# yisol/IDM-VTON

Measured on AMD Instinct MI355X. Metric: try-on images/sec at 768x1024, 30 DDIM steps, guidance 2.0, higher is better.
Workload: dtype bf16; 1 GPU; BASELINE.json configs[1]: 768x1024, 30 steps, batch 2/GPU, guidance 2.0, bf16 storage / fp32 accumulate, scheduler ddim, hipGraph on, GarmentNet batched over 6 timesteps, GarmentNet(block b+1)||TryonNet(block b) two-stream overlap on; images_per_call=2, parallelism=dp1 (image shards, one start-up RCCL weight broadcast), rccl_ranks=1

## Files before the change

### idm-vton_amd/csrc/norm.hip

```cpp
#include <cstdlib>
#include "common.cuh"

template <typename T, int NCH, bool X32, int RPW>
__global__ __launch_bounds__(256) void layernorm_kernel(const idmvton_layernorm_args a) {
    typedef typename VT<T>::v8 v8;
    const int lane = threadIdx.x & 63;
    const int row0 = (blockIdx.x * 4 + (threadIdx.x >> 6)) * RPW;
    if (row0 >= a.rows) return;
    const int nchunk = a.C >> 3;
    const T* gamma = (const T*)a.gamma;
    const T* beta = (const T*)a.beta;
    v8 gm[NCH], bt_[NCH];
#pragma unroll
    for (int i = 0; i < NCH; ++i) {
        const int c = lane + 64 * i;
        if (c < nchunk) { gm[i] = *(const v8*)(gamma + c * 8); bt_[i] = *(const v8*)(beta + c * 8); }
    }
    float v[RPW][NCH][8];
    float s[RPW];
#pragma unroll
    for (int r = 0; r < RPW; ++r) {
        const int row = row0 + r < a.rows ? row0 + r : a.rows - 1;
        const T* x = (const T*)a.x + (size_t)row * a.ldx;
        const float* xf = (const float*)a.x + (size_t)row * a.ldx;
// ... 92 lines not shown
template <typename T, bool X32> struct GnLoad {
    typedef typename VT<T>::v8 v8;
    struct raw { v8 t; };
    static __device__ __forceinline__ raw ld(const void* base, size_t idx) { raw r; r.t = *(const v8*)((const T*)base + idx); return r; }
    static __device__ __forceinline__ float get(const raw& r, int j) { return (float)r.t[j]; }
};
template <typename T> struct GnLoad<T, true> {
    struct raw { float4 a, b; };
    static __device__ __forceinline__ raw ld(const void* base, size_t idx) {
        raw r; const float4* p = (const float4*)((const float*)base + idx); r.a = p[0]; r.b = p[1]; return r;
    }
    static __device__ __forceinline__ float get(const raw& r, int j) {
        return j == 0 ? r.a.x : j == 1 ? r.a.y : j == 2 ? r.a.z : j == 3 ? r.a.w : j == 4 ? r.b.x : j == 5 ? r.b.y : j == 6 ? r.b.z : r.b.w;
    }
};

template <typename T, bool X32>
__global__ __launch_bounds__(256) void gn_stats_kernel(const idmvton_groupnorm_args a, int pix_per_block, int nblk) {
    typedef GnLoad<T, X32> L;
    __shared__ float red_s[GN_MAXC], red_q[GN_MAXC];
    const int b = blockIdx.y;
    const int nchunk = a.C >> 3;
    const int tpp = 256 / nchunk > 0 ? 256 / nchunk : 1;
    const int chunk = threadIdx.x % nchunk, psub = threadIdx.x / nchunk;
    const int p0 = blockIdx.x * pix_per_block;
    const int p1 = min(p0 + pix_per_block, a.HW);
    for (int cb = chunk; cb < nchunk; cb += 256) {
        const int c0 = cb * 8;
        const void* src; int pitch, coff;
        if (c0 < a.C1) { src = a.x; pitch = a.C1; coff = c0; }
        else { src = a.x2; pitch = a.C - a.C1; coff = c0 - a.C1; }
        float s[8], q[8];
#pragma unroll
        for (int j = 0; j < 8; ++j) { s[j] = 0.f; q[j] = 0.f; }
        if (psub < tpp) {
            int pix = p0 + psub;
            for (; pix + 3 * tpp < p1; pix += 4 * tpp) {
                typename L::raw t[4];
#pragma unroll
                for (int u4 = 0; u4 < 4; ++u4) t[u4] = L::ld(src, ((size_t)b * a.HW + pix + u4 * tpp) * pitch + coff);
#pragma unroll
                for (int u4 = 0; u4 < 4; ++u4)
#pragma unroll
                    for (int j = 0; j < 8; ++j) { const float f = L::get(t[u4], j); s[j] += f; q[j] += f * f; }
            }
            for (; pix < p1; pix += tpp) {
                const typename L::raw t = L::ld(src, ((size_t)b * a.HW + pix) * pitch + coff);
#pragma unroll
                for (int j = 0; j < 8; ++j) { const float f = L::get(t, j); s[j] += f; q[j] += f * f; }
            }
#pragma unroll
            for (int j = 0; j < 8; ++j) { red_s[psub * a.C + c0 + j] = s[j]; red_q[psub * a.C + c0 + j] = q[j]; }
        }
    }
    __syncthreads();
    for (int c = threadIdx.x; c < a.C; c += 256) {
        float ss = red_s[c], qq = red_q[c];
        for (int p = 1; p < tpp; ++p) { ss += red_s[p * a.C + c]; qq += red_q[p * a.C + c]; }
        red_s[c] = ss; red_q[c] = qq;
    }
    __syncthreads();
    const int cpg = a.C / a.groups;
    double* part = a.stats + (size_t)2 * a.B * a.groups;
    for (int g = threadIdx.x; g < a.groups; g += 256) {
        double ds = 0.0, dq = 0.0;
        for (int c = g * cpg; c < (g + 1) * cpg; ++c) { ds += (double)red_s[c]; dq += (double)red_q[c]; }
        double* dst = part + (((size_t)b * a.groups + g) * nblk + blockIdx.x) * 2;
        dst[0] = ds; dst[1] = dq;
    }
}

__global__ __launch_bounds__(64) void gn_finalize_kernel(double* stats, int bg, int nblk, double cnt, double eps) {
    const int i = blockIdx.x, lane = threadIdx.x;
    const double* part = stats + (size_t)2 * bg + (size_t)i * nblk * 2;
    double ds = 0.0, dq = 0.0;
    int k = lane;
    for (; k + 3 * 64 < nblk; k += 4 * 64) {
        double ps[4], pq[4];
#pragma unroll
        for (int u4 = 0; u4 < 4; ++u4) { ps[u4] = part[2 * (k + 64 * u4)]; pq[u4] = part[2 * (k + 64 * u4) + 1]; }
#pragma unroll
        for (int u4 = 0; u4 < 4; ++u4) { ds += ps[u4]; dq += pq[u4]; }
    }
    for (; k < nblk; k += 64) { ds += part[2 * k]; dq += part[2 * k + 1]; }
#pragma unroll
    for (int o = 32; o > 0; o >>= 1) { ds += __shfl_xor(ds, o); dq += __shfl_xor(dq, o); }
    if (lane == 0) {
        const double mean = ds / cnt;
        double var = dq / cnt - mean * mean;
        var = var > 0.0 ? var : 0.0;
        float* o = (float*)(stats + 2 * i);
        o[0] = (float)mean;
        o[1] = (float)(1.0 / sqrt(var + eps));
    }
}

template <typename T, bool PREC>
__global__ __launch_bounds__(256) void gn_apply_kernel(const idmvton_groupnorm_args a, int pix_per_block) {
    typedef typename VT<T>::v8 v8;
    typedef GnLoad<T, PREC> L;
    const int b = blockIdx.y;
    const int nchunk = a.C >> 3;
    const int tpp = 256 / nchunk > 0 ? 256 / nchunk : 1;
    const int chunk = threadIdx.x % nchunk, psub = threadIdx.x / nchunk;
    const int p0 = blockIdx.x * pix_per_block;
    const int p1 = min(p0 + pix_per_block, a.HW);
    const int cpg = a.C / a.groups;
    const int opitch = PREC ? 2 * a.C : a.C;
    for (int cb = chunk; cb < nchunk; cb += 256) {
        const int c0 = cb * 8;
        const void* src; int pitch, coff;
        if (c0 < a.C1) { src = a.x; pitch = a.C1; coff = c0; }
        else { src = a.x2; pitch = a.C - a.C1; coff = c0 - a.C1; }
        float sc[8], sh[8];
#pragma unroll
        for (int j = 0; j < 8; ++j) {
            const int c = c0 + j, g = c / cpg;
            const float2 mr = *(const float2*)(a.stats + ((size_t)b * a.groups + g) * 2);
            const float gm = PREC ? ((const float*)a.gamma)[c] : (float)((const T*)a.gamma)[c];
            const float bt = PREC ? ((const float*)a.beta)[c] : (float)((const T*)a.beta)[c];
            sc[j] = mr.y * gm;
            sh[j] = bt - mr.x * sc[j];
        }
        auto emit = [&](const typename L::raw& t, size_t row) {
            T* dst = (T*)a.y + row * opitch + c0;
            v8 o, lo;
#pragma unroll
            for (int j = 0; j < 8; ++j) {
                float f = L::get(t, j) * sc[j] + sh[j];
                if (a.silu) f = silu_f(f);
                o[j] = (T)f;
                if constexpr (PREC) lo[j] = (T)(f - (float)o[j]);
            }
            *(v8*)dst = o;
            if constexpr (PREC) *(v8*)(dst + a.C) = lo;
        };
        if (psub < tpp) {
            int pix = p0 + psub;
            for (; pix + 3 * tpp < p1; pix += 4 * tpp) {
                typename L::raw t[4];
#pragma unroll
                for (int u4 = 0; u4 < 4; ++u4) t[u4] = L::ld(src, ((size_t)b * a.HW + pix + u4 * tpp) * pitch + coff);
#pragma unroll
                for (int u4 = 0; u4 < 4; ++u4) emit(t[u4], (size_t)b * a.HW + pix + u4 * tpp);
            }
            for (; pix < p1; pix += tpp) {
                const size_t row = (size_t)b * a.HW + pix;
                emit(L::ld(src, row * pitch + coff), row);
            }
        }
    }
}

static void gn_geometry(const idmvton_groupnorm_args& a, int& nblk, int& ppb) {
    nblk = (2048 + a.B - 1) / a.B;
    ppb = (a.HW + nblk - 1) / nblk;
    const int nchunk = a.C >> 3;
    const int tpp = 256 / nchunk > 0 ? 256 / nchunk : 1;
    if (ppb < tpp * 4) ppb = tpp * 4;
    nblk = (a.HW + ppb - 1) / ppb;
}

template <typename T>
static int launch_gn(const idmvton_groupnorm_args& a, hipStream_t st) {
    int nblk, ppb;
    gn_geometry(a, nblk, ppb);
    const dim3 grid(nblk, a.B), block(256);
    const bool prec = a.flags != 0;
    if (prec) hipLaunchKernelGGL((gn_stats_kernel<T, true>), grid, block, 0, st, a, ppb, nblk);
    else hipLaunchKernelGGL((gn_stats_kernel<T, false>), grid, block, 0, st, a, ppb, nblk);
    hipLaunchKernelGGL(gn_finalize_kernel, dim3(a.B * a.groups), dim3(64), 0, st, a.stats, a.B * a.groups, nblk,
                       (double)(a.C / a.groups) * (double)a.HW, (double)a.eps);
    if (prec) hipLaunchKernelGGL((gn_apply_kernel<T, true>), grid, block, 0, st, a, ppb);
    else hipLaunchKernelGGL((gn_apply_kernel<T, false>), grid, block, 0, st, a, ppb);
    CHECK_LAUNCH("groupnorm");
    return IDMVTON_OK;
}

extern "C" int idmvton_groupnorm_stats_doubles(int B, int HW, int C, int groups) {
    if (B <= 0 || HW <= 0 || C < 8 || groups <= 0) return -1;
    idmvton_groupnorm_args a;
    a.B = B; a.HW = HW; a.C = C; a.groups = groups;
    int nblk, ppb;
    gn_geometry(a, nblk, ppb);
    return 2 * B * groups * (1 + nblk);
}

extern "C" int idmvton_groupnorm(const idmvton_groupnorm_args* a, void* stream) {
    CHECK_ARG(a != nullptr, IDMVTON_E_ARG, "groupnorm: null args");
    CHECK_ARG(a->dtype == IDMVTON_F16 || a->dtype == IDMVTON_BF16, IDMVTON_E_DTYPE, "groupnorm: dtype %d", a->dtype);
    CHECK_ARG(a->B > 0 && a->HW > 0 && a->C > 0 && a->groups > 0 && a->C % a->groups == 0 && a->C % 8 == 0 && a->C <= GN_MAXC,
              IDMVTON_E_SHAPE, "groupnorm: B=%d HW=%d C=%d groups=%d", a->B, a->HW, a->C, a->groups);
    CHECK_ARG(a->x && a->y && a->gamma && a->beta && a->stats, IDMVTON_E_ARG, "groupnorm: null pointer");
    CHECK_ARG(a->stats_doubles >= idmvton_groupnorm_stats_doubles(a->B, a->HW, a->C, a->groups), IDMVTON_E_SHAPE,
              "groupnorm: stats scratch holds %d doubles, needs %d", a->stats_doubles,
              idmvton_groupnorm_stats_doubles(a->B, a->HW, a->C, a->groups));
    CHECK_ARG(a->C1 > 0 && a->C1 <= a->C && a->C1 % 8 == 0 && (a->C1 == a->C || a->x2), IDMVTON_E_SHAPE, "groupnorm: C1=%d", a->C1);
    constexpr int PREC_FLAGS = IDMVTON_GN_X_F32 | IDMVTON_GN_Y_SPLIT | IDMVTON_GN_AFFINE_F32;
    CHECK_ARG(a->flags == 0 || a->flags == PREC_FLAGS, IDMVTON_E_ARG, "groupnorm: flags=%d (0, or the split-precision form X_F32 | Y_SPLIT | AFFINE_F32 = %d)", a->flags, PREC_FLAGS);
    if (a->flags) CHECK_ARG((((uintptr_t)a->gamma | (uintptr_t)a->beta) & 3) == 0, IDMVTON_E_ALIGN, "groupnorm: fp32 gamma / beta alignment");
    CHECK_ARG((((uintptr_t)a->x | (uintptr_t)a->x2 | (uintptr_t)a->y) & 15) == 0, IDMVTON_E_ALIGN, "groupnorm: pointer alignment");
    return a->dtype == IDMVTON_BF16 ? launch_gn<bf16_t>(*a, (hipStream_t)stream) : launch_gn<f16_t>(*a, (hipStream_t)stream);
}

template <typename T>
__global__ __launch_bounds__(256) void softmax_rows_kernel(T* x, int n, int ld, float scale, int nv) {
    typedef typename VT<T>::v8 v8;
    __shared__ float red[8];
    T* row = x + (size_t)blockIdx.x * ld;
    const int nchunk = n >> 3;
    const float sl = scale * 1.44269504088896341f;
    float mx = -3.0e38f;
    for (int c = threadIdx.x; c < nchunk; c += 256) {
        const v8 t = *(const v8*)(row + c * 8);
#pragma unroll
        for (int j = 0; j < 8; ++j) mx = fmaxf(mx, c * 8 + j < nv ? (float)t[j] : -3.0e38f);
    }
#pragma unroll
    for (int o = 32; o > 0; o >>= 1) mx = fmaxf(mx, __shfl_xor(mx, o));
    if ((threadIdx.x & 63) == 0) red[threadIdx.x >> 6] = mx;
    __syncthreads();
    mx = fmaxf(fmaxf(red[0], red[1]), fmaxf(red[2], red[3]));
    __syncthreads();
    float s = 0.f;
    for (int c = threadIdx.x; c < nchunk; c += 256) {
        const v8 t = *(const v8*)(row + c * 8);
#pragma unroll
        for (int j = 0; j < 8; ++j) s += c * 8 + j < nv ? __builtin_amdgcn_exp2f(((float)t[j] - mx) * sl) : 0.f;
    }
    s = wave_sum(s);
    if ((threadIdx.x & 63) == 0) red[4 + (threadIdx.x >> 6)] = s;
    __syncthreads();
    const float inv = 1.0f / (red[4] + red[5] + red[6] + red[7]);
    for (int c = threadIdx.x; c < nchunk; c += 256) {
        const v8 t = *(const v8*)(row + c * 8);
        v8 o;
#pragma unroll
        for (int j = 0; j < 8; ++j) o[j] = (T)(c * 8 + j < nv ? __builtin_amdgcn_exp2f(((float)t[j] - mx) * sl) * inv : 0.f);
        *(v8*)(row + c * 8) = o;
    }
}

template <typename T>
__global__ __launch_bounds__(256) void softmax_rows_split_kernel(const float* x, int n, int ld, float scale, T* y, int ldy, int nv) {
    typedef typename VT<T>::v8 v8;
    __shared__ float red[8];
    const float* row = x + (size_t)blockIdx.x * ld;
    T* yr = y + (size_t)blockIdx.x * ldy;
    const int nchunk = n >> 3;
    const float sl = scale * 1.44269504088896341f;
    float mx = -3.0e38f;
    for (int c = threadIdx.x; c < nchunk; c += 256) {
        const float4 t0 = *(const float4*)(row + c * 8), t1 = *(const float4*)(row + c * 8 + 4);
        const float v[8] = {t0.x, t0.y, t0.z, t0.w, t1.x, t1.y, t1.z, t1.w};
#pragma unroll
        for (int j = 0; j < 8; ++j) mx = fmaxf(mx, c * 8 + j < nv ? v[j] : -3.0e38f);
    }
#pragma unroll
    for (int o = 32; o > 0; o >>= 1) mx = fmaxf(mx, __shfl_xor(mx, o));
    if ((threadIdx.x & 63) == 0) red[threadIdx.x >> 6] = mx;
    __syncthreads();
    mx = fmaxf(fmaxf(red[0], red[1]), fmaxf(red[2], red[3]));
    __syncthreads();
    float s = 0.f;
    for (int c = threadIdx.x; c < nchunk; c += 256) {
        const float4 t0 = *(const float4*)(row + c * 8), t1 = *(const float4*)(row + c * 8 + 4);
        const float v[8] = {t0.x, t0.y, t0.z, t0.w, t1.x, t1.y, t1.z, t1.w};
#pragma unroll
        for (int j = 0; j < 8; ++j) s += c * 8 + j < nv ? __builtin_amdgcn_exp2f((v[j] - mx) * sl) : 0.f;
    }
    s = wave_sum(s);
    if ((threadIdx.x & 63) == 0) red[4 + (threadIdx.x >> 6)] = s;
    __syncthreads();
    const float inv = 1.0f / (red[4] + red[5] + red[6] + red[7]);
    for (int c = threadIdx.x; c < nchunk; c += 256) {
        const float4 t0 = *(const float4*)(row + c * 8), t1 = *(const float4*)(row + c * 8 + 4);
        const float v[8] = {t0.x, t0.y, t0.z, t0.w, t1.x, t1.y, t1.z, t1.w};
        v8 hi, lo;
#pragma unroll
        for (int j = 0; j < 8; ++j) {
            const float p = c * 8 + j < nv ? __builtin_amdgcn_exp2f((v[j] - mx) * sl) * inv : 0.f;
            hi[j] = (T)p;
            lo[j] = (T)(p - (float)hi[j]);
        }
        *(v8*)(yr + c * 8) = hi;
        *(v8*)(yr + n + c * 8) = lo;
    }
}

extern "C" int idmvton_softmax_rows(const idmvton_softmax_args* a, void* stream) {
    CHECK_ARG(a && a->x, IDMVTON_E_ARG, "softmax_rows: null pointer");
    CHECK_ARG(a->dtype == IDMVTON_F16 || a->dtype == IDMVTON_BF16, IDMVTON_E_DTYPE, "softmax_rows: dtype %d", a->dtype);
    CHECK_ARG(a->rows > 0 && a->n > 0 && a->n % 8 == 0 && (a->y_split || a->ld % 8 == 0) && a->ld >= a->n && ((uintptr_t)a->x & 15) == 0,
              IDMVTON_E_SHAPE, "softmax_rows: rows=%d n=%d ld=%d", a->rows, a->n, a->ld);
    const dim3 grid(a->rows), block(256);
    CHECK_ARG(a->n_valid >= 0 && a->n_valid <= a->n, IDMVTON_E_SHAPE, "softmax_rows: n_valid=%d n=%d", a->n_valid, a->n);
    const int nv = a->n_valid ? a->n_valid : a->n;
    if (a->y_split) {
        CHECK_ARG(a->ldy % 8 == 0 && a->ldy >= 2 * a->n && ((uintptr_t)a->y_split & 15) == 0 && a->ld % 4 == 0, IDMVTON_E_SHAPE, "softmax_rows: y_split ldy=%d n=%d", a->ldy, a->n);
        if (a->dtype == IDMVTON_BF16) hipLaunchKernelGGL((softmax_rows_split_kernel<bf16_t>), grid, block, 0, (hipStream_t)stream, (const float*)a->x, a->n, a->ld, a->scale, (bf16_t*)a->y_split, a->ldy, nv);
        else hipLaunchKernelGGL((softmax_rows_split_kernel<f16_t>), grid, block, 0, (hipStream_t)stream, (const float*)a->x, a->n, a->ld, a->scale, (f16_t*)a->y_split, a->ldy, nv);
        CHECK_LAUNCH("softmax_rows");
        return IDMVTON_OK;
    }
    if (a->dtype == IDMVTON_BF16) hipLaunchKernelGGL((softmax_rows_kernel<bf16_t>), grid, block, 0, (hipStream_t)stream, (bf16_t*)a->x, a->n, a->ld, a->scale, nv);
    else hipLaunchKernelGGL((softmax_rows_kernel<f16_t>), grid, block, 0, (hipStream_t)stream, (f16_t*)a->x, a->n, a->ld, a->scale, nv);
    CHECK_LAUNCH("softmax_rows");
    return IDMVTON_OK;
}
```

### idm-vton_amd/ffi.py

```python
import ctypes as C
import functools
import os

_HERE = os.path.dirname(os.path.abspath(__file__))
LIB_PATH = os.environ.get("IDMVTON_HIP_LIB") or os.path.join(_HERE, "libidmvton_hip.so")

F16, BF16, F32, F8E4M3 = 0, 1, 2, 3
EPI_NONE, EPI_GEGLU, EPI_GELU, EPI_QUICKGELU, EPI_XATTN = 0, 1, 2, 3, 4
ATTN_SELF, ATTN_CROSS = 0, 1
IO_RES_F32, IO_OUT_F32, IO_BIAS_F32, IO_OUT_F8 = 1, 2, 4, 8
GN_X_F32, GN_Y_SPLIT, GN_AFFINE_F32 = 1, 2, 4
LAYOUT_SPLIT, LAYOUT_NHWC_F32 = 1, 2
SPLIT_ACT, SPLIT_W3, SPLIT_W3T = 0, 1, 2
KVS_WIDEN_E4M3, KVS_COPY = 0, 1
MAX_SEG = 24
ABI_VERSION = 9

i32, u32, f32, vp = C.c_int32, C.c_uint32, C.c_float, C.c_void_p


class Seg(C.Structure):
    _fields_ = [("ptr", vp), ("bytes", u32), ("pitch", i32), ("coff", i32), ("len", i32), ("dy", i32), ("dx", i32)]


class XAttn(C.Structure):
    _fields_ = [("nseg", i32), ("k", vp * 2), ("ldk", i32 * 2), ("k_rows", i32 * 2), ("vt", vp * 2), ("ldvt", i32 * 2), ("nk", i32 * 2),
                ("tokens", i32), ("ip_scale", f32)]


class GemmConvArgs(C.Structure):
    _fields_ = [("dtype", i32), ("w", vp), ("N", i32), ("Ktot", i32), ("nseg", i32), ("seg", Seg * MAX_SEG),
                ("M", i32), ("Ho", i32), ("Wo", i32), ("Hi", i32), ("Wi", i32), ("stride", i32), ("ups", i32),
                ("out", vp), ("ldo", i32), ("bias", vp), ("rowbias", vp), ("rowbias_ld", i32),
                ("rows_per_group", i32), ("res", vp), ("ldr", i32), ("mode", i32), ("vt", vp), ("vt_n0", i32),
                ("vt_tokens", i32), ("tile_hint", i32), ("vt_perm", i32), ("io_flags", i32), ("xattn", C.POINTER(XAttn)),
                ("colscale_n", i32), ("colscale", f32), ("f8_out_scale", f32), ("f8_vt_scale", f32)]


class AttnArgs(C.Structure):
    _fields_ = [("dtype", i32), ("mode", i32), ("B", i32), ("heads", i32), ("Nq", i32), ("q", vp), ("ldq", i32),
                ("out", vp), ("ldo", i32), ("nseg", i32), ("k", vp * 2), ("ldk", i32 * 2), ("vt", vp * 2),
                ("ldvt", i32 * 2), ("nk", i32 * 2), ("k_rows", i32 * 2), ("seg_b0", i32 * 2), ("ip_scale", f32), ("tune", i32), ("q_prescaled", i32)]


class LayerNormArgs(C.Structure):
    _fields_ = [("dtype", i32), ("rows", i32), ("C", i32), ("x", vp), ("ldx", i32), ("gamma", vp), ("beta", vp),
                ("eps", f32), ("y", vp), ("ldy", i32), ("y2", vp), ("ldy2", i32), ("x_f32", i32)]


class GroupNormArgs(C.Structure):
    _fields_ = [("dtype", i32), ("B", i32), ("HW", i32), ("C", i32), ("groups", i32), ("x", vp), ("C1", i32),
                ("x2", vp), ("gamma", vp), ("beta", vp), ("eps", f32), ("silu", i32), ("y", vp), ("stats", vp), ("stats_doubles", i32),
                ("flags", i32)]


class PackInputArgs(C.Structure):
    _fields_ = [("dtype", i32), ("B", i32), ("hw", i32), ("cpad", i32), ("latents", vp), ("cond", vp), ("out", vp)]


class CfgStepArgs(C.Structure):
    _fields_ = [("dtype", i32), ("B", i32), ("hw", i32), ("ldc", i32), ("eps_nhwc", vp), ("latents", vp),
                ("noise", vp), ("coef", vp)]


class LayoutArgs(C.Structure):
    _fields_ = [("dtype", i32), ("B", i32), ("C", i32), ("HW", i32), ("cpad", i32), ("to_nhwc", i32), ("src", vp),
                ("dst", vp), ("scale", f32), ("shift", f32), ("flags", i32)]


class VaeSampleArgs(C.Structure):
    _fields_ = [("dtype", i32), ("B", i32), ("hw", i32), ("ldm", i32), ("moments", vp), ("noise", vp), ("z", vp),
                ("scale", f32)]


class AttnSmallArgs(C.Structure):
    _fields_ = [("dtype", i32), ("B", i32), ("heads", i32), ("Lq", i32), ("Lk", i32), ("d", i32), ("q", vp), ("ldq", i32),
                ("k", vp), ("ldk", i32), ("v", vp), ("ldv", i32), ("out", vp), ("ldo", i32), ("scale", f32), ("causal", i32)]


class AttnF8Args(C.Structure):
    _fields_ = [("out_dtype", i32), ("B", i32), ("heads", i32), ("Nq", i32), ("q8", vp), ("ldq", i32), ("out", vp), ("ldo", i32),
                ("nseg", i32), ("k8", vp * 2), ("ldk", i32 * 2), ("vt8", vp * 2), ("ldvt", i32 * 2), ("nk", i32 * 2), ("k_rows", i32 * 2),
                ("seg_b0", i32 * 2), ("qk_scale_exp", i32), ("v_scale_exp", i32)]


class QuantF8Args(C.Structure):
    _fields_ = [("dtype", i32), ("mode", i32), ("rows", i32), ("cols", i32), ("src", vp), ("lds", i32), ("dst", vp), ("ldd", i32), ("scale", f32)]


class SoftmaxArgs(C.Structure):
    _fields_ = [("dtype", i32), ("rows", i32), ("n", i32), ("ld", i32), ("x", vp), ("scale", f32), ("y_split", vp), ("ldy", i32), ("n_valid", i32)]


class SplitArgs(C.Structure):
    _fields_ = [("dtype", i32), ("mode", i32), ("rows", i32), ("cols", i32), ("src", vp), ("lds", i32), ("dst", vp), ("ldd", i32)]


class KvUnpackDesc(C.Structure):
    _fields_ = [("src", vp), ("dst", vp), ("exp", vp), ("rows", i32), ("cols", i32), ("lds", i32), ("ldd", i32)]


class KvUnpackArgs(C.Structure):
    _fields_ = [("dtype", i32), ("n", i32), ("desc", vp), ("max_chunks", i32)]


class KvStreamDesc(KvUnpackDesc):
    pass


class KvStreamArgs(C.Structure):
    _fields_ = [("dtype", i32), ("mode", i32), ("n", i32), ("workgroups", i32), ("desc", vp), ("first", vp)]


STRUCTS = {"idmvton_seg": Seg, "idmvton_gemm_conv_args": GemmConvArgs, "idmvton_attn_args": AttnArgs,
           "idmvton_layernorm_args": LayerNormArgs, "idmvton_groupnorm_args": GroupNormArgs,
           "idmvton_pack_input_args": PackInputArgs, "idmvton_cfg_step_args": CfgStepArgs,
           "idmvton_layout_args": LayoutArgs, "idmvton_vae_sample_args": VaeSampleArgs, "idmvton_softmax_args": SoftmaxArgs,
           "idmvton_attn_small_args": AttnSmallArgs, "idmvton_attn_f8_args": AttnF8Args, "idmvton_quant_f8_args": QuantF8Args,
           "idmvton_split_args": SplitArgs, "idmvton_xattn": XAttn, "idmvton_kv_unpack_desc": KvUnpackDesc,
           "idmvton_kv_unpack_args": KvUnpackArgs, "idmvton_kv_stream_desc": KvStreamDesc, "idmvton_kv_stream_args": KvStreamArgs}

SYMBOLS = ["idmvton_last_error", "idmvton_abi_version", "idmvton_sizeof", "idmvton_gemm_conv", "idmvton_attn_fwd",
           "idmvton_layernorm", "idmvton_groupnorm", "idmvton_pack_input", "idmvton_cfg_step", "idmvton_layout",
           "idmvton_vae_sample", "idmvton_softmax_rows", "idmvton_probe_mfma", "idmvton_groupnorm_stats_doubles",
           "idmvton_attn_small", "idmvton_rccl_unique_id", "idmvton_rccl_comm_init", "idmvton_rccl_bcast_arena",
           "idmvton_rccl_comm_destroy", "idmvton_attn_f8", "idmvton_quant_f8", "idmvton_split", "idmvton_attn_fwd_shared",
           "idmvton_attn_f8_shared", "idmvton_attn_fwd_indexed", "idmvton_attn_f8_indexed",
           "idmvton_attn_fwd_ragged", "idmvton_attn_f8_ragged", "idmvton_kv_unpack", "idmvton_kv_stream",
           "idmvton_host_device_ptr", "idmvton_kv_fill", "idmvton_kv_place"]

_lib = None


class HipLibraryMissing(RuntimeError):
    pass


def lib():
    global _lib
    if _lib is not None:
        return _lib
    if not os.path.exists(LIB_PATH):
        raise HipLibraryMissing(f"{LIB_PATH} not built: run `make -C {os.path.join(_HERE, 'csrc')}` "
                                "(or __graft_entry__.build()); there is no CPU fallback")
    L = C.CDLL(LIB_PATH)
    for s in SYMBOLS:
        if not hasattr(L, s):
            raise HipLibraryMissing(f"{LIB_PATH} does not export {s}")
    L.idmvton_last_error.restype = C.c_char_p
    L.idmvton_sizeof.argtypes = [C.c_char_p]
    L.idmvton_abi_version.restype = C.c_int
    v = L.idmvton_abi_version()
    if v != ABI_VERSION:
        raise HipLibraryMissing(f"{LIB_PATH} implements C ABI version {v}, this binding needs {ABI_VERSION}: rebuild it "
                                f"(`make -C {os.path.join(_HERE, 'csrc')}`)")
    for name, st in STRUCTS.items():
        n = L.idmvton_sizeof(name.encode())
        if n != C.sizeof(st):
            raise HipLibraryMissing(f"ABI drift: sizeof({name}) is {n} in the library, {C.sizeof(st)} in ffi.py")
    for s in ("idmvton_gemm_conv", "idmvton_attn_fwd", "idmvton_layernorm", "idmvton_groupnorm",
              "idmvton_pack_input", "idmvton_cfg_step", "idmvton_layout", "idmvton_vae_sample", "idmvton_softmax_rows",
              "idmvton_attn_small", "idmvton_attn_f8", "idmvton_quant_f8", "idmvton_split"):
        getattr(L, s).argtypes = [vp, vp]
        getattr(L, s).restype = C.c_int
# ... 91 lines not shown
```

### idm-vton_amd/ops.py

```python
import ctypes as C
import json
import os

import torch

from . import ffi

_DT = {torch.float16: ffi.F16, torch.bfloat16: ffi.BF16}


def _dt(t):
    try:
        return _DT[t.dtype]
    except KeyError:
        raise TypeError(f"idm_vton_amd ops take float16/bfloat16 tensors, got {t.dtype}") from None


def _stream():
    return torch.cuda.current_stream().cuda_stream


PROFILE = None


# ... 314 lines not shown
        self.slices = [(0, self.n)] if slices is None else [(int(f), int(c)) for f, c in slices]
        for f, c in self.slices:
            if f % 2 or f < 0 or c < 1 or c > KV_STREAM_MAX_N or f + c > self.n:
                raise ValueError(f"kv_stream: descriptors [{f}, {f + c}) of {self.n} (an even first index, 1 to {KV_STREAM_MAX_N} descriptors)")
        self.items = kv_items(self.host)
        firsts = [kv_stream_first(self.items[f:f + c]) for f, c in self.slices]
        self.first_at, at = [], 0
        for t in firsts:
            self.first_at.append(at)
            at += t.numel()
        self.first_host = torch.cat(firsts).contiguous()
        self.dev, self.first_dev = self.host.to(device), self.first_host.to(device)

    def launch(self, dtype, which=0, workgroups=None):
        f0, c = self.slices[which]
        a = ffi.KvStreamArgs()
        a.dtype, a.mode, a.n, a.workgroups = _DT[dtype], self.mode, c, KV_STREAM_WORKGROUPS if workgroups is None else workgroups
        a.desc, a.first = self.dev.data_ptr() + 40 * f0, self.first_dev.data_ptr() + 4 * self.first_at[which]
        call = getattr(ffi, "call_" + self.ENTRY)
        launch = lambda: call(a, self.host.data_ptr() + 40 * f0, self.first_host.data_ptr() + 4 * self.first_at[which], _stream())
        if PROFILE is None:
            return launch()
        e0, e1 = torch.cuda.Event(enable_timing=True), torch.cuda.Event(enable_timing=True)
        e0.record()
        launch()
        e1.record()
        PROFILE.append(("idmvton_" + self.ENTRY, e0, e1, 0.0, self.bytes_moved(f0, c)))

    def bytes_moved(self, f0, c):
        return (48.0 if self.mode == ffi.KVS_WIDEN_E4M3 else 32.0) * float(self.items[f0:f0 + c].sum())


class KvFillTable(KvStreamTable):
    ENTRY = "kv_fill"

    def link_bytes(self, f0=0, c=None):
        c = self.n - f0 if c is None else c
        return 16.0 * float(self.items[f0:f0 + c][self.host[f0:f0 + c, 0] != 0].sum())

    def bytes_moved(self, f0, c):
        return self.link_bytes(f0, c) + (32.0 if self.mode == ffi.KVS_WIDEN_E4M3 else 16.0) * float(self.items[f0:f0 + c].sum())


class KvPlaceTable(KvFillTable):
    ENTRY = "kv_place"

    def launch(self, dtype, which=0, workgroups=None):
        return super().launch(dtype, which, 0)


def kv_pad_even(rec):
    if rec.shape[0] % 2 == 0:
        return rec
    m = int(kv_items(rec).argmin())
    return torch.cat([rec, rec[m:m + 1]])


def _kv_table(cls, descs, dtype, mode, device):
    if isinstance(descs, KvStreamTable):
        return descs
    widen, zero_ok = mode == ffi.KVS_WIDEN_E4M3, cls is not KvStreamTable
    rec = []
    for src, dst, exp in descs:
        ok = dst.dim() == 2 and dst.stride(1) == 1 and dst.is_cuda and (not widen or dst.dtype == dtype) and (zero_ok or src is not None)
        if ok and src is not None:
            ok = src.dim() == 2 and src.shape == dst.shape and src.stride(1) == 1
            if widen:
                ok = ok and src.dtype == torch.uint8 and exp is not None and exp.dtype == torch.int32 and exp.numel() == 1
            else:
                ok = ok and src.dtype == dst.dtype
        if not ok:
            raise ValueError("%s: a run is (uint8 [rows][cols], %s [rows][cols], one int32) when widening, (x [rows][cols], x [rows][cols], None) "
                             "when copying%s; rows contiguous, the destination on the device"
                             % (cls.ENTRY, dtype, ", (None, dst [rows][cols], None) for a zero run" if zero_ok else ""))
        rows, cols = dst.shape
        sz = 1 if widen else dst.element_size()
        if src is None:
            rec.append((0, _ptr(dst), 0, rows | ((cols * sz) << 32), (cols * sz) | ((dst.stride(0) * sz) << 32)))
        else:
            rec.append((stream_address(src), _ptr(dst), stream_address(exp) if widen else 0, rows | ((cols * sz) << 32),
                        (src.stride(0) * sz) | ((dst.stride(0) * sz) << 32)))
    device = descs[0][1].device if device is None else device
    return cls(torch.tensor(rec, dtype=torch.int64).reshape(-1, 5), device, mode)


def kv_stream(descs, dtype, mode=ffi.KVS_WIDEN_E4M3, workgroups=None, device=None):
    descs = _kv_table(KvStreamTable, descs, dtype, mode, device)
    descs.launch(dtype, 0, workgroups)
    return descs


def kv_fill(descs, dtype, mode=ffi.KVS_WIDEN_E4M3, workgroups=None, device=None):
    descs = _kv_table(KvFillTable, descs, dtype, mode, device)
    descs.launch(dtype, 0, workgroups)
    return descs


def kv_place(descs, dtype, mode=ffi.KVS_WIDEN_E4M3, device=None):
    descs = _kv_table(KvPlaceTable, descs, dtype, mode, device)
    descs.launch(dtype, 0)
    return descs


def attention_f8(q8, out, segs, heads, *, qk_scale_exp, v_scale_exp, B, Nq, ldq=None, ldo=None):
    a = ffi.AttnF8Args()
    a.out_dtype, a.B, a.heads, a.Nq = _dt(out), B, heads, Nq
    a.q8, a.ldq = _ptr(q8), (q8.stride(-2) if ldq is None else ldq)
    a.out, a.ldo = _ptr(out), (out.stride(-2) if ldo is None else ldo)
    a.nseg = len(segs)
    fl = 0.0
    for i, s in enumerate(segs):
        a.k8[i], a.vt8[i] = _ptr(s["k8"]), _ptr(s["vt8"])
        a.ldk[i], a.ldvt[i] = s["ldk"], s["ldvt"]
        a.nk[i], a.k_rows[i], a.seg_b0[i] = s["nk"], s.get("k_rows", 0), s.get("b0", 0)
        fl += 4.0 * (B - s.get("b0", 0)) * heads * Nq * s["nk"] * 64
    a.qk_scale_exp, a.v_scale_exp = qk_scale_exp, v_scale_exp
    nb, ix, nkt = _seg_nb(segs), _seg_index(segs, B), _seg_nk(segs, B)
    _call("idmvton_attn_f8_ragged" if nkt else "idmvton_attn_f8_indexed" if ix else "idmvton_attn_f8_shared" if nb else "idmvton_attn_f8", a, flops=fl,
          bytes_=float(B * Nq * heads * 64 * (1 + out.element_size())), seg_nb=nb or ([0, 0] if ix or nkt else None), seg_index=ix, seg_nk=nkt)
    return out


def attention_small(q, k, v, out, heads, d, *, scale, causal=False, B=None, Lq=None, Lk=None, ldq=None, ldk=None, ldv=None, ldo=None):
    a = ffi.AttnSmallArgs()
    a.dtype = _dt(q)
    a.B = q.shape[0] if B is None else B
    a.heads, a.d = heads, d
    a.Lq = q.shape[1] if Lq is None else Lq
    a.Lk = k.shape[1] if Lk is None else Lk
    a.q, a.ldq = _ptr(q), (q.stride(-2) if ldq is None else ldq)
    a.k, a.ldk = _ptr(k), (k.stride(-2) if ldk is None else ldk)
    a.v, a.ldv = _ptr(v), (v.stride(-2) if ldv is None else ldv)
    a.out, a.ldo = _ptr(out), (out.stride(-2) if ldo is None else ldo)
    a.scale, a.causal = scale, int(bool(causal))
    _call("idmvton_attn_small", a, flops=4.0 * a.B * heads * a.Lq * a.Lk * d)
    return out


def layernorm(x, gamma, beta, eps=1e-5, out=None, out2=None):
    rows, Cc = x.shape
    if out is None:
        out = torch.empty((rows, Cc), dtype=gamma.dtype, device=x.device)
    a = ffi.LayerNormArgs()
    a.dtype, a.rows, a.C = _dt(gamma), rows, Cc
    a.x_f32 = int(x.dtype == torch.float32)
    a.x, a.ldx = _ptr(x), x.stride(0)
    a.gamma, a.beta, a.eps = _ptr(gamma), _ptr(beta), eps
    a.y, a.ldy = _ptr(out), out.stride(0)
    a.y2, a.ldy2 = _ptr(out2), (out2.stride(0) if out2 is not None else 0)
    _call("idmvton_layernorm", a, bytes_=(x.element_size() + (1.0 + (out2 is not None)) * out.element_size()) * rows * Cc)
    return out


def groupnorm(x, gamma, beta, groups, eps, silu, stats, x2=None, out=None, split_dtype=None):
    B, HW, C1 = x.shape
    Cc = C1 + (x2.shape[-1] if x2 is not None else 0)
    prec = split_dtype is not None
    if prec and not (x.dtype == gamma.dtype == beta.dtype == torch.float32 and (x2 is None or x2.dtype == torch.float32)):
        raise TypeError("groupnorm(split_dtype=...): x, gamma and beta must be float32")
    if out is None:
        out = torch.empty((B, HW, 2 * Cc if prec else Cc), dtype=split_dtype if prec else x.dtype, device=x.device)
    a = ffi.GroupNormArgs()
    a.dtype, a.B, a.HW, a.C, a.groups = _dt(out), B, HW, Cc, groups
    a.flags = (ffi.GN_X_F32 | ffi.GN_Y_SPLIT | ffi.GN_AFFINE_F32) if prec else 0
    a.x, a.C1, a.x2 = _ptr(x), C1, _ptr(x2)
    a.gamma, a.beta, a.eps, a.silu = _ptr(gamma), _ptr(beta), eps, int(bool(silu))
    a.y, a.stats, a.stats_doubles = _ptr(out), _ptr(stats), stats.numel()
    _call("idmvton_groupnorm", a, bytes_=(2.0 * x.element_size() + (2 if prec else 1) * out.element_size()) * B * HW * Cc)
    return out


GN_STATS_DOUBLES = 2 * 32 * (2048 + 2 * 64 + 64)


def gn_stats_doubles(B, HW, C, groups):
    return ffi.lib().idmvton_groupnorm_stats_doubles(B, HW, C, groups)


def pack_input(latents, cond, out):
    a = ffi.PackInputArgs()
    B, hw = latents.shape[0], latents.shape[2] * latents.shape[3] if latents.dim() == 4 else latents.shape[2]
    a.dtype, a.B, a.hw, a.cpad = _dt(out), B, hw, out.shape[-1]
    a.latents, a.cond, a.out = _ptr(latents), _ptr(cond), _ptr(out)
    _call("idmvton_pack_input", a)
    return out


def cfg_step(eps_nhwc, latents, noise, coef):
    a = ffi.CfgStepArgs()
    B = latents.shape[0]
    hw = latents.numel() // (B * 4)
    a.dtype, a.B, a.hw, a.ldc = _dt(eps_nhwc), B, hw, eps_nhwc.shape[-1]
    a.eps_nhwc, a.latents, a.noise, a.coef = _ptr(eps_nhwc), _ptr(latents), _ptr(noise), _ptr(coef)
    _call("idmvton_cfg_step", a)
    return latents


def to_nhwc(src_nchw_f32, dtype, cpad=None, scale=1.0, shift=0.0, out=None, split=False):
    B, Cc = src_nchw_f32.shape[:2]
    HW = src_nchw_f32.numel() // (B * Cc)
    cpad = Cc if cpad is None else cpad
    if out is None:
        out = torch.empty((B, HW, 2 * cpad if split else cpad), dtype=dtype, device=src_nchw_f32.device)
    a = ffi.LayoutArgs()
    a.flags = ffi.LAYOUT_SPLIT if split else 0
    a.dtype, a.B, a.C, a.HW, a.cpad, a.to_nhwc = _dt(out), B, Cc, HW, cpad, 1
    a.src, a.dst, a.scale, a.shift = _ptr(src_nchw_f32), _ptr(out), scale, shift
    _call("idmvton_layout", a)
    return out


def to_nchw(src_nhwc, Cc, shape_hw, scale=1.0, shift=0.0, out=None):
    B, HW, cpad = src_nhwc.shape
    if out is None:
        out = torch.empty((B, Cc) + tuple(shape_hw), dtype=torch.float32, device=src_nhwc.device)
    a = ffi.LayoutArgs()
    f32 = src_nhwc.dtype == torch.float32
    a.flags = ffi.LAYOUT_NHWC_F32 if f32 else 0
    a.dtype, a.B, a.C, a.HW, a.cpad, a.to_nhwc = (ffi.BF16 if f32 else _dt(src_nhwc)), B, Cc, HW, cpad, 0
    a.src, a.dst, a.scale, a.shift = _ptr(src_nhwc), _ptr(out), scale, shift
    _call("idmvton_layout", a)
    return out


def vae_sample(moments_nhwc, noise, scale, out=None):
    B, hw, ldm = moments_nhwc.shape
    if out is None:
        out = torch.empty_like(noise)
    a = ffi.VaeSampleArgs()
    a.dtype, a.B, a.hw, a.ldm = _dt(moments_nhwc), B, hw, ldm
    a.moments, a.noise, a.z, a.scale = _ptr(moments_nhwc), _ptr(noise), _ptr(out), scale
    _call("idmvton_vae_sample", a)
    return out


def softmax_rows(x, scale, n_valid=0):
    a = ffi.SoftmaxArgs()
    a.dtype, a.rows, a.n, a.ld = _dt(x), x.shape[0], x.shape[1], x.stride(0)
    a.x, a.scale, a.n_valid = _ptr(x), scale, n_valid
    _call("idmvton_softmax_rows", a)
    return x


def softmax_rows_split(x, scale, dtype, n_valid=0, out=None):
    rows, n = x.shape
    if out is None:
        out = torch.empty((rows, 2 * n), dtype=dtype, device=x.device)
    elif tuple(out.shape) != (rows, 2 * n) or out.dtype != dtype:
        raise ValueError(f"softmax_rows_split(out=...): needs shape {(rows, 2 * n)} of {dtype}, got {tuple(out.shape)} of {out.dtype}")
    a = ffi.SoftmaxArgs()
    a.n_valid = n_valid
    a.dtype, a.rows, a.n, a.ld = _dt(out), rows, n, x.stride(0)
    a.x, a.scale, a.y_split, a.ldy = _ptr(x), scale, _ptr(out), out.stride(0)
    _call("idmvton_softmax_rows", a, bytes_=float(rows * n * (3 * 4 + 2 * out.element_size())))
    return out


def split(x, dtype, mode=ffi.SPLIT_ACT, out=None):
    rows, cols = x.shape
    shape = {ffi.SPLIT_ACT: (rows, 2 * cols), ffi.SPLIT_W3: (rows, 3 * cols), ffi.SPLIT_W3T: (cols, 3 * rows)}[mode]
    if out is None:
        out = torch.empty(shape, dtype=dtype, device=x.device)
    elif tuple(out.shape) != shape or out.dtype != dtype:
        raise ValueError(f"split(out=...): needs shape {shape} of {dtype}, got {tuple(out.shape)} of {out.dtype}")
    a = ffi.SplitArgs()
    a.dtype, a.mode, a.rows, a.cols = _dt(out), mode, rows, cols
    a.src, a.lds, a.dst, a.ldd = _ptr(x), x.stride(0), _ptr(out), out.stride(0)
    _call("idmvton_split", a, bytes_=float(rows * cols * 4 + out.numel() * out.element_size()))
    return out


def probe_mfma(which, a, b):
    c = torch.empty((64, 16), dtype=torch.float32, device=a.device)
    rc = ffi.lib().idmvton_probe_mfma(which, C.c_void_p(a.data_ptr()), C.c_void_p(b.data_ptr()),
                                      C.c_void_p(c.data_ptr()), C.c_void_p(_stream()))
    if rc != 0:
        raise RuntimeError(ffi.lib().idmvton_last_error().decode())
    return c


load_tune()
```

### include/idmvton_hip.h

```cpp
#ifndef IDMVTON_HIP_H
#define IDMVTON_HIP_H
#include <stddef.h>
#include <stdint.h>

#ifdef __cplusplus
extern "C" {
#endif

enum { IDMVTON_OK = 0, IDMVTON_E_SHAPE = -1, IDMVTON_E_DTYPE = -2, IDMVTON_E_ALIGN = -3, IDMVTON_E_LAUNCH = -4,
       IDMVTON_E_ARG = -5 };
enum { IDMVTON_F16 = 0, IDMVTON_BF16 = 1, IDMVTON_F32 = 2, IDMVTON_F8E4M3 = 3  };

const char* idmvton_last_error(void);
int idmvton_abi_version(void);
int idmvton_sizeof(const char* struct_name);

#define IDMVTON_MAX_SEG 24
typedef struct {
    const void* ptr;
    uint32_t bytes;
    int32_t pitch;
    int32_t coff;
    int32_t len;
    int32_t dy, dx;
} idmvton_seg;

enum { IDMVTON_EPI_NONE = 0, IDMVTON_EPI_GEGLU = 1, IDMVTON_EPI_GELU = 2 ,
       IDMVTON_EPI_QUICKGELU = 3 ,
       IDMVTON_EPI_XATTN = 4  };
typedef struct {
    int32_t nseg;
    const void* k[2]; int32_t ldk[2]; int32_t k_rows[2];
    const void* vt[2]; int32_t ldvt[2];
    int32_t nk[2];
    int32_t tokens; float ip_scale;
} idmvton_xattn;
enum { IDMVTON_IO_RES_F32 = 1, IDMVTON_IO_OUT_F32 = 2, IDMVTON_IO_BIAS_F32 = 4, IDMVTON_IO_OUT_F8 = 8 };
typedef struct {
    int32_t dtype;
    const void* w; int32_t N; int32_t Ktot;
    int32_t nseg; idmvton_seg seg[IDMVTON_MAX_SEG];
    int32_t M, Ho, Wo, Hi, Wi, stride, ups;
    void* out; int32_t ldo;
    const void* bias;
    const void* rowbias; int32_t rowbias_ld; int32_t rows_per_group;
    const void* res; int32_t ldr;
    int32_t mode;
    void* vt; int32_t vt_n0; int32_t vt_tokens;
    int32_t tile_hint;
    int32_t vt_perm;
    int32_t io_flags;
    const idmvton_xattn* xattn;
    int32_t colscale_n; float colscale;
    float f8_out_scale, f8_vt_scale;
} idmvton_gemm_conv_args;
int idmvton_gemm_conv(const idmvton_gemm_conv_args* a, void* stream);

enum { IDMVTON_ATTN_SELF = 0, IDMVTON_ATTN_CROSS = 1 };
typedef struct {
    int32_t dtype; int32_t mode;
    int32_t B, heads, Nq;
    const void* q; int32_t ldq;
    void* out; int32_t ldo;
    int32_t nseg;
    const void* k[2]; int32_t ldk[2];
    const void* vt[2]; int32_t ldvt[2];
    int32_t nk[2];
    int32_t k_rows[2];
    int32_t seg_b0[2];
    float ip_scale;
    int32_t tune;
    int32_t q_prescaled;
} idmvton_attn_args;
int idmvton_attn_fwd(const idmvton_attn_args* a, void* stream);
int idmvton_attn_fwd_shared(const idmvton_attn_args* a, const int32_t seg_nb[2], void* stream);
int idmvton_attn_fwd_indexed(const idmvton_attn_args* a, const int32_t seg_nb[2], const int32_t* const seg_index[2], void* stream);
int idmvton_attn_fwd_ragged(const idmvton_attn_args* a, const int32_t seg_nb[2], const int32_t* const seg_index[2],
                            const int32_t* const seg_nk[2], void* stream);

typedef struct {
    int32_t out_dtype; int32_t B, heads, Nq;
    const void* q8; int32_t ldq;
    void* out; int32_t ldo;
    int32_t nseg;
    const void* k8[2]; int32_t ldk[2];
    const void* vt8[2]; int32_t ldvt[2];
    int32_t nk[2]; int32_t k_rows[2]; int32_t seg_b0[2];
    int32_t qk_scale_exp; int32_t v_scale_exp;
} idmvton_attn_f8_args;
int idmvton_attn_f8(const idmvton_attn_f8_args* a, void* stream);
int idmvton_attn_f8_shared(const idmvton_attn_f8_args* a, const int32_t seg_nb[2], void* stream);
int idmvton_attn_f8_indexed(const idmvton_attn_f8_args* a, const int32_t seg_nb[2], const int32_t* const seg_index[2], void* stream);
int idmvton_attn_f8_ragged(const idmvton_attn_f8_args* a, const int32_t seg_nb[2], const int32_t* const seg_index[2],
                           const int32_t* const seg_nk[2], void* stream);
typedef struct {
    int32_t dtype; int32_t mode; int32_t rows, cols;
    const void* src; int32_t lds;
    void* dst; int32_t ldd;
    float scale;
} idmvton_quant_f8_args;
int idmvton_quant_f8(const idmvton_quant_f8_args* a, void* stream);

typedef struct {
    const void* src;
    void* dst;
    const int32_t* exp;
    int32_t rows, cols, lds, ldd;
} idmvton_kv_unpack_desc;
typedef struct {
    int32_t dtype; int32_t n;
    const idmvton_kv_unpack_desc* desc;
    int32_t max_chunks;
} idmvton_kv_unpack_args;
int idmvton_kv_unpack(const idmvton_kv_unpack_args* a, const idmvton_kv_unpack_desc* host_desc, void* stream);

enum { IDMVTON_KVS_WIDEN_E4M3 = 0, IDMVTON_KVS_COPY = 1 };
#define IDMVTON_KVS_MAX_N (1 << 20)
typedef idmvton_kv_unpack_desc idmvton_kv_stream_desc;
typedef struct {
    int32_t dtype; int32_t mode; int32_t n; int32_t workgroups;
    const idmvton_kv_stream_desc* desc;
    const int32_t* first;
} idmvton_kv_stream_args;
int idmvton_kv_stream(const idmvton_kv_stream_args* a, const idmvton_kv_stream_desc* host_desc, const int32_t* host_first, void* stream);
int idmvton_host_device_ptr(const void* host, void** dev);

int idmvton_kv_fill(const idmvton_kv_stream_args* a, const idmvton_kv_stream_desc* host_desc, const int32_t* host_first, void* stream);

int idmvton_kv_place(const idmvton_kv_stream_args* a, const idmvton_kv_stream_desc* host_desc, const int32_t* host_first, void* stream);

typedef struct {
    int32_t dtype; int32_t B, heads, Lq, Lk, d;
    const void* q; int32_t ldq;
    const void* k; int32_t ldk;
    const void* v; int32_t ldv;
    void* out; int32_t ldo;
    float scale; int32_t causal;
} idmvton_attn_small_args;
int idmvton_attn_small(const idmvton_attn_small_args* a, void* stream);

typedef struct {
    int32_t dtype; int32_t rows, C;
    const void* x; int32_t ldx;
    const void* gamma; const void* beta; float eps;
    void* y; int32_t ldy;
    void* y2; int32_t ldy2;
    int32_t x_f32;
} idmvton_layernorm_args;
int idmvton_layernorm(const idmvton_layernorm_args* a, void* stream);

enum { IDMVTON_GN_X_F32 = 1 , IDMVTON_GN_Y_SPLIT = 2 ,
       IDMVTON_GN_AFFINE_F32 = 4  };
typedef struct {
    int32_t dtype; int32_t B, HW, C, groups;
    const void* x; int32_t C1;
    const void* x2;
    const void* gamma; const void* beta; float eps; int32_t silu;
    void* y;
    double* stats; int32_t stats_doubles;
    int32_t flags;
} idmvton_groupnorm_args;
int idmvton_groupnorm(const idmvton_groupnorm_args* a, void* stream);
int idmvton_groupnorm_stats_doubles(int B, int HW, int C, int groups);

typedef struct {
    int32_t dtype; int32_t B, hw, cpad;
    const float* latents; const void* cond; void* out;
} idmvton_pack_input_args;
int idmvton_pack_input(const idmvton_pack_input_args* a, void* stream);

typedef struct {
    int32_t dtype; int32_t B, hw, ldc;
    const void* eps_nhwc; float* latents; const float* noise; const float* coef;
} idmvton_cfg_step_args;
int idmvton_cfg_step(const idmvton_cfg_step_args* a, void* stream);

enum { IDMVTON_LAYOUT_SPLIT = 1 , IDMVTON_LAYOUT_NHWC_F32 = 2  };
typedef struct {
    int32_t dtype; int32_t B, C, HW, cpad; int32_t to_nhwc;
    const void* src; void* dst; float scale; float shift;
    int32_t flags;
} idmvton_layout_args;
int idmvton_layout(const idmvton_layout_args* a, void* stream);

typedef struct {
    int32_t dtype; int32_t B, hw, ldm;
    const void* moments; const float* noise; float* z; float scale;
} idmvton_vae_sample_args;
int idmvton_vae_sample(const idmvton_vae_sample_args* a, void* stream);

typedef struct {
    int32_t dtype; int32_t rows, n, ld;
    void* x; float scale;
    void* y_split; int32_t ldy;
    int32_t n_valid;
} idmvton_softmax_args;
int idmvton_softmax_rows(const idmvton_softmax_args* a, void* stream);

enum { IDMVTON_SPLIT_ACT = 0, IDMVTON_SPLIT_W3 = 1, IDMVTON_SPLIT_W3T = 2 };
typedef struct {
    int32_t dtype; int32_t mode; int32_t rows, cols;
    const float* src; int32_t lds;
    void* dst; int32_t ldd;
} idmvton_split_args;
int idmvton_split(const idmvton_split_args* a, void* stream);

int idmvton_rccl_unique_id(void* id128);
int idmvton_rccl_comm_init(const void* id128, int rank, int world, void** comm_out);
int idmvton_rccl_bcast_arena(void* comm, void* buf, uint64_t bytes, int root, uint64_t chunk_bytes, void* stream);
int idmvton_rccl_comm_destroy(void* comm);

int idmvton_probe_mfma(int which, const void* a, const void* b, float* c, void* stream);

#ifdef __cplusplus
}
#endif
#endif
```

Baseline: 1.578 images/s.

## Add single-kernel register-resident GroupNorm path for small group slabs

Adds a one-pass GroupNorm kernel that gives each (batch, group) its own 512-thread block. The block holds the whole group slab in registers and computes the mean and a centred variance with DPP wave reductions in fp64, then applies affine and SiLU from those registers. It replaces the three-launch stats/finalize/apply path whenever the slab fits, removing the second read of the activations and two extra launches. The grid is only B*groups blocks, so large-HW groups may underuse the GPU. A NO_SLAB flag is added to force the old path.

```diff
diff --git a/idm-vton_amd/csrc/norm.hip b/idm-vton_amd/csrc/norm.hip
--- a/idm-vton_amd/csrc/norm.hip
+++ b/idm-vton_amd/csrc/norm.hip
@@ -268,6 +268,155 @@
     }
 }
 
+#define GN_SLAB_NT 512
+#define GN_SLAB_BYTES 256
+template <typename T, int VW> struct GnSlabVec;
+template <typename T> struct GnSlabVec<T, 8> { typedef u32x4 raw; typedef typename VT<T>::v8 vec; };
+template <typename T> struct GnSlabVec<T, 4> { typedef u32x2 raw; typedef typename VT<T>::v4 vec; };
+
+template <int CTRL> __device__ __forceinline__ double dpp_f64(double v) {
+    const uint2 u = __builtin_bit_cast(uint2, v);
+    uint2 r;
+    r.x = __builtin_amdgcn_update_dpp(0, u.x, CTRL, 0xf, 0xf, false);
+    r.y = __builtin_amdgcn_update_dpp(0, u.y, CTRL, 0xf, 0xf, false);
+    return __builtin_bit_cast(double, r);
+}
+__device__ __forceinline__ double readlane_f64(double v, int lane) {
+    const uint2 u = __builtin_bit_cast(uint2, v);
+    uint2 r;
+    r.x = __builtin_amdgcn_readlane(u.x, lane);
+    r.y = __builtin_amdgcn_readlane(u.y, lane);
+    return __builtin_bit_cast(double, r);
+}
+__device__ __forceinline__ double wave_sum_dpp_f64(double v) {
+    v += dpp_f64<0xb1>(v);
+    v += dpp_f64<0x4e>(v);
+    v += dpp_f64<0x141>(v);
+    v += dpp_f64<0x140>(v);
+    return (readlane_f64(v, 0) + readlane_f64(v, 16)) + (readlane_f64(v, 32) + readlane_f64(v, 48));
+}
+__device__ __forceinline__ double gn_slab_total(double part, double* red) {
+    const double w = wave_sum_dpp_f64(part);
+    if ((threadIdx.x & 63) == 0) red[threadIdx.x >> 6] = w;
+    __syncthreads();
+    return ((red[0] + red[1]) + (red[2] + red[3])) + ((red[4] + red[5]) + (red[6] + red[7]));
+}
+template <int VW> __device__ __forceinline__ float gn_fold(const float (&s)[VW]) {
+    if constexpr (VW == 8) return ((s[0] + s[1]) + (s[2] + s[3])) + ((s[4] + s[5]) + (s[6] + s[7]));
+    else return (s[0] + s[1]) + (s[2] + s[3]);
+}
+
+template <typename T, int VW, int NV>
+__global__ __launch_bounds__(GN_SLAB_NT, 4) void gn_slab_kernel(const idmvton_groupnorm_args a) {
+    typedef typename GnSlabVec<T, VW>::raw raw;
+    typedef typename GnSlabVec<T, VW>::vec vec;
+    __shared__ double red[2][GN_SLAB_NT / 64];
+    const int lin = xcd_remap(blockIdx.x, gridDim.x);
+    const int b = lin / a.groups, g = lin - b * a.groups;
+    const int cpg = a.C / a.groups, vpp = cpg / VW, tpp = GN_SLAB_NT / vpp;
+    const int chunk = threadIdx.x % vpp, psub = threadIdx.x / vpp;
+    const bool live = psub < tpp;
+    const int cg = g * cpg;
+    const T* src; int pitch, coff;
+    if (cg < a.C1) { src = (const T*)a.x; pitch = a.C1; coff = cg; }
+    else { src = (const T*)a.x2; pitch = a.C - a.C1; coff = cg - a.C1; }
+    const T* xp = src + (size_t)b * a.HW * pitch + coff + chunk * VW;
+    raw v[NV];
+#pragma unroll
+    for (int i = 0; i < NV; ++i) {
+        const int pix = psub + i * tpp;
+        if (live && pix < a.HW) v[i] = *(const raw*)(xp + (size_t)pix * pitch);
+    }
+    raw gm_r = {}, bt_r = {};
+    if (live) { gm_r = *(const raw*)((const T*)a.gamma + cg + chunk * VW); bt_r = *(const raw*)((const T*)a.beta + cg + chunk * VW); }
+    const double cnt = (double)cpg * (double)a.HW;
+    float s[VW];
+    double acc = 0.0;
+#pragma unroll
+    for (int i = 0; i < NV; ++i) {
+        if (live && psub + i * tpp < a.HW) {
+            const vec t = __builtin_bit_cast(vec, v[i]);
+#pragma unroll
+            for (int j = 0; j < VW; ++j) s[j] = (float)t[j];
+            acc += (double)gn_fold<VW>(s);
+        }
+    }
+    const double mean = gn_slab_total(acc, red[0]) / cnt;
+    const float mf = (float)mean;
+#pragma unroll
+    for (int i = 0; i < NV; ++i) asm volatile("" : "+v"(v[i]));
+    acc = 0.0;
+#pragma unroll
+    for (int i = 0; i < NV; ++i) {
+        if (live && psub + i * tpp < a.HW) {
+            const vec t = __builtin_bit_cast(vec, v[i]);
+#pragma unroll
+            for (int j = 0; j < VW; ++j) { const float d = (float)t[j] - mf; s[j] = d * d; }
+            acc += (double)gn_fold<VW>(s);
+        }
+    }
+    const double dm = mean - (double)mf;
+    double var = gn_slab_total(acc, red[1]) / cnt - dm * dm;
+    var = var > 0.0 ? var : 0.0;
+    const float rstd = (float)(1.0 / sqrt(var + (double)a.eps));
+    if (!live) return;
+#pragma unroll
+    for (int i = 0; i < NV; ++i) asm volatile("" : "+v"(v[i]));
+    const vec gm = __builtin_bit_cast(vec, gm_r), bt = __builtin_bit_cast(vec, bt_r);
+    float sc[VW], sh[VW];
+#pragma unroll
+    for (int j = 0; j < VW; ++j) {
+        sc[j] = rstd * (float)gm[j];
+        sh[j] = (float)bt[j] - mf * sc[j];
+    }
+    T* yp = (T*)a.y + (size_t)b * a.HW * a.C + cg + chunk * VW;
+#pragma unroll
+    for (int i = 0; i < NV; ++i) {
+        const int pix = psub + i * tpp;
+        if (pix < a.HW) {
+            const vec t = __builtin_bit_cast(vec, v[i]);
+            vec o;
+#pragma unroll
+            for (int j = 0; j < VW; ++j) {
+                float f = (float)t[j] * sc[j] + sh[j];
+                if (a.silu) f = silu_f(f);
+                o[j] = (T)f;
+            }
+            *(raw*)(yp + (size_t)pix * a.C) = __builtin_bit_cast(raw, o);
+        }
+    }
+}
+
+static int gn_slab_tpp(const idmvton_groupnorm_args& a, int esz, int& vw, int& nv) {
+    if (a.flags != 0) return 0;
+    const int cpg = a.C / a.groups;
+    if (cpg % 4 != 0) return 0;
+    if (a.C1 != a.C && a.C1 % cpg != 0) return 0;
+    vw = cpg % 8 == 0 ? 8 : 4;
+    const int vpp = cpg / vw;
+    if (vpp > GN_SLAB_NT) return 0;
+    if ((((uintptr_t)a.gamma | (uintptr_t)a.beta) & (uintptr_t)(vw * esz - 1)) != 0) return 0;
+    const int tpp = GN_SLAB_NT / vpp, nvmax = GN_SLAB_BYTES / (vw * esz);
+    const int need = (a.HW + tpp - 1) / tpp;
+    if (need > nvmax) return 0;
+    nv = 1;
+    while (nv < need) nv *= 2;
+    return tpp;
+}
+
+template <typename T, int VW>
+static void launch_gn_slab(const idmvton_groupnorm_args& a, int nv, hipStream_t st) {
+    const dim3 grid(a.B * a.groups), block(GN_SLAB_NT);
+    switch (nv) {
+        case 1: hipLaunchKernelGGL((gn_slab_kernel<T, VW, 1>), grid, block, 0, st, a); break;
+        case 2: hipLaunchKernelGGL((gn_slab_kernel<T, VW, 2>), grid, block, 0, st, a); break;
+        case 4: hipLaunchKernelGGL((gn_slab_kernel<T, VW, 4>), grid, block, 0, st, a); break;
+        case 8: hipLaunchKernelGGL((gn_slab_kernel<T, VW, 8>), grid, block, 0, st, a); break;
+        case 16: hipLaunchKernelGGL((gn_slab_kernel<T, VW, 16>), grid, block, 0, st, a); break;
+        default: hipLaunchKernelGGL((gn_slab_kernel<T, VW, 256 / (VW * 2)>), grid, block, 0, st, a); break;
+    }
+}
+
 static void gn_geometry(const idmvton_groupnorm_args& a, int& nblk, int& ppb) {
     nblk = (2048 + a.B - 1) / a.B;
     ppb = (a.HW + nblk - 1) / nblk;
@@ -279,10 +428,17 @@
 
 template <typename T>
 static int launch_gn(const idmvton_groupnorm_args& a, hipStream_t st) {
+    int vw = 0, nv = 0;
+    if (gn_slab_tpp(a, (int)sizeof(T), vw, nv)) {
+        if (vw == 8) launch_gn_slab<T, 8>(a, nv, st);
+        else launch_gn_slab<T, 4>(a, nv, st);
+        CHECK_LAUNCH("groupnorm");
+        return IDMVTON_OK;
+    }
     int nblk, ppb;
     gn_geometry(a, nblk, ppb);
     const dim3 grid(nblk, a.B), block(256);
-    const bool prec = a.flags != 0;
+    const bool prec = (a.flags & ~IDMVTON_GN_NO_SLAB) != 0;
     if (prec) hipLaunchKernelGGL((gn_stats_kernel<T, true>), grid, block, 0, st, a, ppb, nblk);
     else hipLaunchKernelGGL((gn_stats_kernel<T, false>), grid, block, 0, st, a, ppb, nblk);
     hipLaunchKernelGGL(gn_finalize_kernel, dim3(a.B * a.groups), dim3(64), 0, st, a.stats, a.B * a.groups, nblk,
@@ -313,8 +469,9 @@
               idmvton_groupnorm_stats_doubles(a->B, a->HW, a->C, a->groups));
     CHECK_ARG(a->C1 > 0 && a->C1 <= a->C && a->C1 % 8 == 0 && (a->C1 == a->C || a->x2), IDMVTON_E_SHAPE, "groupnorm: C1=%d", a->C1);
     constexpr int PREC_FLAGS = IDMVTON_GN_X_F32 | IDMVTON_GN_Y_SPLIT | IDMVTON_GN_AFFINE_F32;
-    CHECK_ARG(a->flags == 0 || a->flags == PREC_FLAGS, IDMVTON_E_ARG, "groupnorm: flags=%d (0, or the split-precision form X_F32 | Y_SPLIT | AFFINE_F32 = %d)", a->flags, PREC_FLAGS);
-    if (a->flags) CHECK_ARG((((uintptr_t)a->gamma | (uintptr_t)a->beta) & 3) == 0, IDMVTON_E_ALIGN, "groupnorm: fp32 gamma / beta alignment");
+    const int form = a->flags & ~IDMVTON_GN_NO_SLAB;
+    CHECK_ARG(form == 0 || form == PREC_FLAGS, IDMVTON_E_ARG, "groupnorm: flags=%d (0, or the split-precision form X_F32 | Y_SPLIT | AFFINE_F32 = %d; either with NO_SLAB = %d)", a->flags, PREC_FLAGS, IDMVTON_GN_NO_SLAB);
+    if (form) CHECK_ARG((((uintptr_t)a->gamma | (uintptr_t)a->beta) & 3) == 0, IDMVTON_E_ALIGN, "groupnorm: fp32 gamma / beta alignment");
     CHECK_ARG((((uintptr_t)a->x | (uintptr_t)a->x2 | (uintptr_t)a->y) & 15) == 0, IDMVTON_E_ALIGN, "groupnorm: pointer alignment");
     return a->dtype == IDMVTON_BF16 ? launch_gn<bf16_t>(*a, (hipStream_t)stream) : launch_gn<f16_t>(*a, (hipStream_t)stream);
 }
diff --git a/idm-vton_amd/ffi.py b/idm-vton_amd/ffi.py
--- a/idm-vton_amd/ffi.py
+++ b/idm-vton_amd/ffi.py
@@ -9,7 +9,7 @@
 EPI_NONE, EPI_GEGLU, EPI_GELU, EPI_QUICKGELU, EPI_XATTN = 0, 1, 2, 3, 4
 ATTN_SELF, ATTN_CROSS = 0, 1
 IO_RES_F32, IO_OUT_F32, IO_BIAS_F32, IO_OUT_F8 = 1, 2, 4, 8
-GN_X_F32, GN_Y_SPLIT, GN_AFFINE_F32 = 1, 2, 4
+GN_X_F32, GN_Y_SPLIT, GN_AFFINE_F32, GN_NO_SLAB = 1, 2, 4, 8
 LAYOUT_SPLIT, LAYOUT_NHWC_F32 = 1, 2
 SPLIT_ACT, SPLIT_W3, SPLIT_W3T = 0, 1, 2
 KVS_WIDEN_E4M3, KVS_COPY = 0, 1
diff --git a/idm-vton_amd/ops.py b/idm-vton_amd/ops.py
--- a/idm-vton_amd/ops.py
+++ b/idm-vton_amd/ops.py
@@ -490,7 +490,7 @@
     return out
 
 
-def groupnorm(x, gamma, beta, groups, eps, silu, stats, x2=None, out=None, split_dtype=None):
+def groupnorm(x, gamma, beta, groups, eps, silu, stats, x2=None, out=None, split_dtype=None, no_slab=False):
     B, HW, C1 = x.shape
     Cc = C1 + (x2.shape[-1] if x2 is not None else 0)
     prec = split_dtype is not None
@@ -500,7 +500,7 @@
         out = torch.empty((B, HW, 2 * Cc if prec else Cc), dtype=split_dtype if prec else x.dtype, device=x.device)
     a = ffi.GroupNormArgs()
     a.dtype, a.B, a.HW, a.C, a.groups = _dt(out), B, HW, Cc, groups
-    a.flags = (ffi.GN_X_F32 | ffi.GN_Y_SPLIT | ffi.GN_AFFINE_F32) if prec else 0
+    a.flags = ((ffi.GN_X_F32 | ffi.GN_Y_SPLIT | ffi.GN_AFFINE_F32) if prec else 0) | (ffi.GN_NO_SLAB if no_slab else 0)
     a.x, a.C1, a.x2 = _ptr(x), C1, _ptr(x2)
     a.gamma, a.beta, a.eps, a.silu = _ptr(gamma), _ptr(beta), eps, int(bool(silu))
     a.y, a.stats, a.stats_doubles = _ptr(out), _ptr(stats), stats.numel()
diff --git a/include/idmvton_hip.h b/include/idmvton_hip.h
--- a/include/idmvton_hip.h
+++ b/include/idmvton_hip.h
@@ -150,7 +150,8 @@
 int idmvton_layernorm(const idmvton_layernorm_args* a, void* stream);
 
 enum { IDMVTON_GN_X_F32 = 1 , IDMVTON_GN_Y_SPLIT = 2 ,
-       IDMVTON_GN_AFFINE_F32 = 4  };
+       IDMVTON_GN_AFFINE_F32 = 4 ,
+       IDMVTON_GN_NO_SLAB = 8  };
 typedef struct {
     int32_t dtype; int32_t B, HW, C, groups;
     const void* x; int32_t C1;
```

Result: no change. 1.585 images/s (median of 6 runs) (+0.4%).
